# opherlieber/rltime

Measured on AMD Instinct MI355X. Metric: sampled transitions/sec (= learner steps/sec x B x T), IQN-LSTM B=512 T=80 84x84x4, higher is better.
Workload: dtype f32

## Files before the change

rltime_amd/csrc/conv_wrw.hip:

```cpp
#include "common.hpp"
#include "split3.hpp"
#include <stdlib.h>

namespace mirl {

typedef float cw_f4 __attribute__((ext_vector_type(4)));

constexpr int CW_F = 64;
constexpr int CW_MAXT = 5;

struct CwArgs {
  const float* x; const float* g; float* partial;
  int N, H, W, C, KH, KW, S, OH, OW;
  int T;
  int NT;
  int FPI;
  int KP;
  int Cp;
  int xplane;
  int gpitch;
};

template <int TPW>
__global__ void __launch_bounds__(512) __attribute__((amdgpu_waves_per_eu(2, 2)))
k_conv_wrw_b3(CwArgs a) {
  extern __shared__ __align__(16) char cw_lds[];
  uint16_t* xs = reinterpret_cast<uint16_t*>(cw_lds);
  uint16_t* gs = xs + 3 * a.xplane;
  int* tbl = reinterpret_cast<int*>(gs + 3 * CW_F * a.gpitch);
  const int tid = threadIdx.x, lane = tid & 63, wave = __builtin_amdgcn_readfirstlane(tid >> 6);
  const int j = lane & 15, kq = lane >> 4;
  const int OHW = a.OH * a.OW, fx = a.H * a.W * a.C, gplane = CW_F * a.gpitch;
  const int ksteps = a.KP >> 5;
  for (int p = tid; p < a.KP; p += 512) {
    const int f = p / OHW, r = p - f * OHW, oh = r / a.OW, ow = r - oh * a.OW;
    tbl[p] = f < a.FPI ? ((f * a.H + a.S * oh) * a.W + a.S * ow) * a.Cp : 0;
  }
  for (int o = tid; o < 3 * a.xplane / 8; o += 512) reinterpret_cast<uint4*>(xs)[o] = make_uint4(0u, 0u, 0u, 0u);
  const int nt0 = wave * TPW;
  int toff[TPW];
#pragma unroll
  for (int i = 0; i < TPW; ++i) {
    int t = (nt0 + i) * 16 + j; if (t > a.T - 1) t = a.T - 1;
    const int c = t % a.C, kk = t / a.C, kw = kk % a.KW, kh = kk / a.KW;
    toff[i] = (kh * a.W + kw) * a.Cp + c;
  }
  g3_f32x4 acc[4][TPW];
#pragma unroll
  for (int m = 0; m < 4; ++m)
#pragma unroll
    for (int i = 0; i < TPW; ++i) acc[m][i] = g3_f32x4{0.f, 0.f, 0.f, 0.f};

  const int units = (a.N + a.FPI - 1) / a.FPI;
  auto put_x = [&](const cw_f4& v, int o) {
    const float q[4] = {v.x, v.y, v.z, v.w};
    uint2 h, m, l;
    g3_split4(q, h, m, l);
    const int pix = (o * 4) / a.C, c0 = o * 4 - pix * a.C;
    uint32_t* d = reinterpret_cast<uint32_t*>(xs + pix * a.Cp + c0);
    d[0] = h.x; d[1] = h.y;
    d[a.xplane / 2] = m.x; d[a.xplane / 2 + 1] = m.y;
    d[a.xplane] = l.x; d[a.xplane + 1] = l.y;
  };
  auto load_g8 = [&](float (&q)[8], const float* gu, int item, int valid_pos) {
    const int f = item & 63, p0 = (item >> 6) * 8;
#pragma unroll
    for (int e = 0; e < 8; ++e) {
      const int p = p0 + e;
      const float t = gu[(int64_t)(p < valid_pos ? p : valid_pos - 1) * CW_F + f];
      q[e] = p < valid_pos ? t : 0.f;
    }
  };
  auto put_g8 = [&](const float (&q)[8], int item) {
    const int f = item & 63, p0 = (item >> 6) * 8;
    const float q0[4] = {q[0], q[1], q[2], q[3]}, q1[4] = {q[4], q[5], q[6], q[7]};
    uint2 h0, m0, l0, h1, m1, l1;
    g3_split4(q0, h0, m0, l0);
    g3_split4(q1, h1, m1, l1);
    uint16_t* d = gs + f * a.gpitch + p0;
    *reinterpret_cast<uint4*>(d) = make_uint4(h0.x, h0.y, h1.x, h1.y);
    *reinterpret_cast<uint4*>(d + gplane) = make_uint4(m0.x, m0.y, m1.x, m1.y);
    *reinterpret_cast<uint4*>(d + 2 * gplane) = make_uint4(l0.x, l0.y, l1.x, l1.y);
  };
  for (int u0 = blockIdx.x; u0 < units; u0 += gridDim.x) {
    const int n0 = u0 * a.FPI;
    const int frames = a.N - n0 < a.FPI ? a.N - n0 : a.FPI;
    const int xv = frames * fx / 4;
    __syncthreads();
    {
      const cw_f4* x4 = reinterpret_cast<const cw_f4*>(a.x + (int64_t)n0 * fx);
      const float* gu = a.g + (int64_t)n0 * OHW * CW_F;
      const int items = (a.KP >> 3) * CW_F, valid_pos = frames * OHW;
      constexpr int LX = 7, LG = 2;
      cw_f4 v[LX];
      float q[LG][8];
#pragma unroll
      for (int k = 0; k < LX; ++k) { const int o = tid + k * 512; v[k] = x4[o < xv ? o : xv - 1]; }
#pragma unroll
      for (int k = 0; k < LG; ++k) { const int it = tid + k * 512; load_g8(q[k], gu, it < items ? it : items - 1, valid_pos); }
#pragma unroll
      for (int k = 0; k < LX; ++k) { const int o = tid + k * 512; if (o < xv) put_x(v[k], o); }
#pragma unroll
      for (int k = 0; k < LG; ++k) { const int it = tid + k * 512; if (it < items) put_g8(q[k], it); }
      for (int o0 = tid + LX * 512; o0 < xv; o0 += 512) put_x(x4[o0], o0);
      for (int it = tid + LG * 512; it < items; it += 512) { float r[8]; load_g8(r, gu, it, valid_pos); put_g8(r, it); }
    }
    __syncthreads();
    for (int ks = 0; ks < ksteps; ++ks) {
      const int p0 = ks * 32 + kq * 8;
      int org[8];
      {
        const int4 t0 = *reinterpret_cast<const int4*>(tbl + p0), t1 = *reinterpret_cast<const int4*>(tbl + p0 + 4);
        org[0] = t0.x; org[1] = t0.y; org[2] = t0.z; org[3] = t0.w; org[4] = t1.x; org[5] = t1.y; org[6] = t1.z; org[7] = t1.w;
      }
      g3_bf16x8 af[4][3];
#pragma unroll
      for (int m = 0; m < 4; ++m)
#pragma unroll
        for (int p = 0; p < 3; ++p)
          af[m][p] = *reinterpret_cast<const g3_bf16x8*>(gs + p * gplane + (16 * m + j) * a.gpitch + p0);
      uint32_t raw[2][3][8];
      auto read_b = [&](uint32_t (&r)[3][8], int i) {
#pragma unroll
        for (int p = 0; p < 3; ++p)
#pragma unroll
          for (int e = 0; e < 8; ++e) r[p][e] = xs[p * a.xplane + org[e] + toff[i]];
      };
      read_b(raw[0], 0);
#pragma unroll
      for (int i = 0; i < TPW; ++i) {
        if (i + 1 < TPW) read_b(raw[(i + 1) & 1], i + 1);
        __builtin_amdgcn_sched_barrier(0);
        g3_bf16x8 bf[3];
#pragma unroll
        for (int p = 0; p < 3; ++p) {
          const uint32_t* r = raw[i & 1][p];
          bf[p] = __builtin_bit_cast(g3_bf16x8, make_uint4(r[0] | (r[1] << 16), r[2] | (r[3] << 16), r[4] | (r[5] << 16), r[6] | (r[7] << 16)));
        }
        constexpr int PA[6] = {2, 0, 1, 1, 0, 0};
        constexpr int PB[6] = {0, 2, 1, 0, 1, 0};
#pragma unroll
        for (int c = 0; c < 6; ++c)
#pragma unroll
          for (int m = 0; m < 4; ++m)
            acc[m][i] = __builtin_amdgcn_mfma_f32_16x16x32_bf16(af[m][PA[c]], bf[PB[c]], acc[m][i], 0, 0, 0);
        __builtin_amdgcn_sched_barrier(0);
      }
    }
  }
  float* out = a.partial + (int64_t)blockIdx.x * CW_F * a.T;
#pragma unroll
  for (int i = 0; i < TPW; ++i) {
    const int t = (nt0 + i) * 16 + j;
    if (nt0 + i < a.NT) {
#pragma unroll
      for (int m = 0; m < 4; ++m)
#pragma unroll
        for (int r = 0; r < 4; ++r) out[(int64_t)(16 * m + 4 * kq + r) * a.T + t] = acc[m][i][r];
    }
  }
}

__global__ void __launch_bounds__(256)
k_conv_wrw_reduce(const cw_f4* __restrict__ partial, int parts, int64_t n4, cw_f4* __restrict__ dw) {
  const int64_t i = (int64_t)blockIdx.x * 256 + threadIdx.x;
  if (i >= n4) return;
  cw_f4 s0 = {0.f, 0.f, 0.f, 0.f}, s1 = s0, s2 = s0, s3 = s0;
  int p = 0;
  for (; p + 4 <= parts; p += 4) {
    s0 += partial[(int64_t)p * n4 + i]; s1 += partial[(int64_t)(p + 1) * n4 + i];
    s2 += partial[(int64_t)(p + 2) * n4 + i]; s3 += partial[(int64_t)(p + 3) * n4 + i];
  }
  for (; p < parts; ++p) s0 += partial[(int64_t)p * n4 + i];
  dw[i] = (s0 + s1) + (s2 + s3);
}

static int cw_geometry(int64_t N, int H, int W, int C, int F, int KH, int KW, int S, CwArgs* a, size_t* lds, unsigned* grid) {
  if (F != CW_F || C < 4 || (C % 4) || KH < 1 || KW < 1 || S < 1 || H < KH || W < KW) return 0;
  const int T = KH * KW * C;
  if (T % 16) return 0;
  const int NT = T / 16;
  if (NT > 8 * CW_MAXT) return 0;
  const int OH = (H - KH) / S + 1, OW = (W - KW) / S + 1, OHW = OH * OW;
  if ((OHW * CW_F) % 4) return 0;
  int best = 0;
  size_t best_lds = 0;
  double best_waste = 0.0;
  for (int fpi = 1; fpi <= 4; ++fpi) {
    const int KP = (fpi * OHW + 31) / 32 * 32;
    const int xplane = (fpi * H * W * (C + 2) + 7) / 8 * 8;
    const size_t need = (size_t)3 * xplane * 2 + (size_t)3 * CW_F * (KP + 8) * 2 + (size_t)KP * 4;
    if (need > 150 * 1024) break;
    const double waste = (double)KP / (fpi * OHW);
    if (!best || waste <= best_waste + 1e-9) { best = fpi; best_lds = need; best_waste = waste; }
  }
  if (!best) return 0;
  if (a) {
    a->N = (int)N; a->H = H; a->W = W; a->C = C; a->KH = KH; a->KW = KW; a->S = S; a->OH = OH; a->OW = OW;
    a->T = T; a->NT = NT; a->FPI = best; a->KP = (best * OHW + 31) / 32 * 32;
    a->Cp = C + 2; a->xplane = (best * H * W * (C + 2) + 7) / 8 * 8; a->gpitch = a->KP + 8;
    const int64_t units = (N + best - 1) / best;
    *grid = (unsigned)(units < 256 ? units : 256);
    *lds = best_lds;
  }
  return 1;
}

}

extern "C" int mirl_conv_wrw_b3_supported(int32_t C, int32_t F, int32_t KH, int32_t KW, int32_t S, int32_t H, int32_t W) {
  return mirl::cw_geometry(1, H, W, C, F, KH, KW, S, nullptr, nullptr, nullptr);
}

extern "C" int mirl_conv_wrw_b3_scratch_bytes(int32_t C, int32_t F, int32_t KH, int32_t KW, int64_t* bytes) {
  if (!bytes || F != mirl::CW_F || C < 1 || KH < 1 || KW < 1) return mirl::fail(MIRL_ERR_ARG, "conv_wrw_b3_scratch_bytes: bad arguments");
  *bytes = (int64_t)256 * F * KH * KW * C * (int64_t)sizeof(float);
  return MIRL_OK;
}

extern "C" int mirl_conv_wrw_b3(int64_t N, int32_t H, int32_t W, int32_t C, int32_t F, int32_t KH, int32_t KW, int32_t S,
                                const float* x, const float* g, void* scratch, int64_t scratch_bytes, float* dw, void* stream) {
  using namespace mirl;
  CwArgs a;
  size_t lds = 0;
  unsigned grid = 0;
  if (N <= 0 || N >= (1LL << 30) || !x || !g || !scratch || !dw) return fail(MIRL_ERR_ARG, "bad conv_wrw_b3 arguments");
  if (!cw_geometry(N, H, W, C, F, KH, KW, S, &a, &lds, &grid)) return fail(MIRL_ERR_ARG, "conv_wrw_b3: unsupported layer shape");
  if (((uintptr_t)x % 16) || ((uintptr_t)g % 16) || ((uintptr_t)scratch % 16) || ((uintptr_t)dw % 16))
    return fail(MIRL_ERR_ARG, "conv_wrw_b3: pointers must be 16-byte aligned");
  if (scratch_bytes < (int64_t)grid * CW_F * a.T * (int64_t)sizeof(float)) return fail(MIRL_ERR_ARG, "conv_wrw_b3: scratch too small");
  a.x = x; a.g = g; a.partial = (float*)scratch;
  hipStream_t st = (hipStream_t)stream;
  const int tpw = (a.NT + 7) / 8;
  const void* fns[CW_MAXT] = {(const void*)k_conv_wrw_b3<1>, (const void*)k_conv_wrw_b3<2>, (const void*)k_conv_wrw_b3<3>,
                              (const void*)k_conv_wrw_b3<4>, (const void*)k_conv_wrw_b3<5>};
  static bool attr[CW_MAXT] = {false, false, false, false, false};
  const void* fn = fns[tpw - 1];
  if (!attr[tpw - 1]) { MIRL_HIP(hipFuncSetAttribute(fn, hipFuncAttributeMaxDynamicSharedMemorySize, 150 * 1024)); attr[tpw - 1] = true; }
  {
    ProfScope ps("k_conv_wrw_b3", 4.0 * (double)N * ((double)H * W * C + (double)a.OH * a.OW * CW_F), st,
                 2.0 * (double)N * a.OH * a.OW * CW_F * a.T);
    void* kargs[] = {(void*)&a};
    MIRL_HIP(hipLaunchKernel(fn, dim3(grid), dim3(512), kargs, lds, st));
  }
  ProfScope ps("k_conv_wrw_reduce", (double)(grid + 1) * CW_F * a.T * 4.0, st);
  const int64_t n4 = (int64_t)CW_F * a.T / 4;
  hipLaunchKernelGGL(k_conv_wrw_reduce, dim3((unsigned)((n4 + 255) / 256)), dim3(256), 0, st, reinterpret_cast<const cw_f4*>(scratch),
                     (int)grid, n4, reinterpret_cast<cw_f4*>(dw));
  MIRL_LAUNCH_CHECK();
  return MIRL_OK;
}
```

Baseline: 481,100.

## Use ds_read_tr16 transposed LDS reads and bank-conflict-aware channel padding in conv wrw

Measured after the change: 484,400 (median of 6 runs). About the same (+0.7%).

```diff
diff --git a/rltime_amd/csrc/conv_wrw.hip b/rltime_amd/csrc/conv_wrw.hip
--- a/rltime_amd/csrc/conv_wrw.hip
+++ b/rltime_amd/csrc/conv_wrw.hip
@@ -8,6 +8,7 @@
 
 constexpr int CW_F = 64;
 constexpr int CW_MAXT = 5;
+constexpr int CW_SLABS = 256;
 
 struct CwArgs {
   const float* x; const float* g; float* partial;
@@ -20,6 +21,14 @@
   int xplane;
   int gpitch;
 };
+
+typedef short cw_i16x4 __attribute__((ext_vector_type(4)));
+
+__device__ __forceinline__ uint2 cw_read_tr(const uint16_t* p) {
+  typedef __attribute__((address_space(3))) cw_i16x4 lds_i16x4;
+  const cw_i16x4 v = __builtin_amdgcn_ds_read_tr16_b64_v4i16((lds_i16x4*)(p));
+  return __builtin_bit_cast(uint2, v);
+}
 
 template <int TPW>
 __global__ void __launch_bounds__(512) __attribute__((amdgpu_waves_per_eu(2, 2)))
@@ -41,7 +50,8 @@
   int toff[TPW];
 #pragma unroll
   for (int i = 0; i < TPW; ++i) {
-    int t = (nt0 + i) * 16 + j; if (t > a.T - 1) t = a.T - 1;
+    const int nt = nt0 + i < a.NT ? nt0 + i : a.NT - 1;
+    const int t = nt * 16 + 4 * (j & 3);
     const int c = t % a.C, kk = t / a.C, kw = kk % a.KW, kh = kk / a.KW;
     toff[i] = (kh * a.W + kw) * a.Cp + c;
   }
@@ -57,10 +67,10 @@
     uint2 h, m, l;
     g3_split4(q, h, m, l);
     const int pix = (o * 4) / a.C, c0 = o * 4 - pix * a.C;
-    uint32_t* d = reinterpret_cast<uint32_t*>(xs + pix * a.Cp + c0);
-    d[0] = h.x; d[1] = h.y;
-    d[a.xplane / 2] = m.x; d[a.xplane / 2 + 1] = m.y;
-    d[a.xplane] = l.x; d[a.xplane + 1] = l.y;
+    uint2* d = reinterpret_cast<uint2*>(xs + pix * a.Cp + c0);
+    d[0] = h;
+    d[a.xplane / 4] = m;
+    d[a.xplane / 2] = l;
   };
   auto load_g8 = [&](float (&q)[8], const float* gu, int item, int valid_pos) {
     const int f = item & 63, p0 = (item >> 6) * 8;
@@ -108,35 +118,27 @@
     __syncthreads();
     for (int ks = 0; ks < ksteps; ++ks) {
       const int p0 = ks * 32 + kq * 8;
-      int org[8];
-      {
-        const int4 t0 = *reinterpret_cast<const int4*>(tbl + p0), t1 = *reinterpret_cast<const int4*>(tbl + p0 + 4);
-        org[0] = t0.x; org[1] = t0.y; org[2] = t0.z; org[3] = t0.w; org[4] = t1.x; org[5] = t1.y; org[6] = t1.z; org[7] = t1.w;
-      }
+      const int o0 = tbl[p0 + (j >> 2)], o1 = tbl[p0 + 4 + (j >> 2)];
       g3_bf16x8 af[4][3];
 #pragma unroll
       for (int m = 0; m < 4; ++m)
 #pragma unroll
         for (int p = 0; p < 3; ++p)
           af[m][p] = *reinterpret_cast<const g3_bf16x8*>(gs + p * gplane + (16 * m + j) * a.gpitch + p0);
-      uint32_t raw[2][3][8];
-      auto read_b = [&](uint32_t (&r)[3][8], int i) {
-#pragma unroll
-        for (int p = 0; p < 3; ++p)
-#pragma unroll
-          for (int e = 0; e < 8; ++e) r[p][e] = xs[p * a.xplane + org[e] + toff[i]];
+      g3_bf16x8 bb[2][3];
+      auto read_b = [&](g3_bf16x8 (&b)[3], int i) {
+#pragma unroll
+        for (int p = 0; p < 3; ++p) {
+          const uint2 lo = cw_read_tr(xs + p * a.xplane + o0 + toff[i]), hi = cw_read_tr(xs + p * a.xplane + o1 + toff[i]);
+          b[p] = __builtin_bit_cast(g3_bf16x8, make_uint4(lo.x, lo.y, hi.x, hi.y));
+        }
       };
-      read_b(raw[0], 0);
+      read_b(bb[0], 0);
 #pragma unroll
       for (int i = 0; i < TPW; ++i) {
-        if (i + 1 < TPW) read_b(raw[(i + 1) & 1], i + 1);
+        if (i + 1 < TPW) read_b(bb[(i + 1) & 1], i + 1);
         __builtin_amdgcn_sched_barrier(0);
-        g3_bf16x8 bf[3];
-#pragma unroll
-        for (int p = 0; p < 3; ++p) {
-          const uint32_t* r = raw[i & 1][p];
-          bf[p] = __builtin_bit_cast(g3_bf16x8, make_uint4(r[0] | (r[1] << 16), r[2] | (r[3] << 16), r[4] | (r[5] << 16), r[6] | (r[7] << 16)));
-        }
+        const g3_bf16x8 (&bf)[3] = bb[i & 1];
         constexpr int PA[6] = {2, 0, 1, 1, 0, 0};
         constexpr int PB[6] = {0, 2, 1, 0, 1, 0};
 #pragma unroll
@@ -175,6 +177,22 @@
   dw[i] = (s0 + s1) + (s2 + s3);
 }
 
+static int cw_read_cycles(int fpi, int H, int W, int S, int OW, int OHW, int KP, int Cp) {
+  int total = 0;
+  for (int p0 = 0; p0 < KP; p0 += 16)
+    for (int sub = 0; sub < 2; ++sub) {
+      int cnt[64] = {0}, worst = 0;
+      for (int k = 0; k < 2; ++k)
+        for (int q = 0; q < 4; ++q) {
+          const int p = p0 + 8 * k + 4 * sub + q, f = p / OHW, r = p - f * OHW, oh = r / OW, ow = r - oh * OW;
+          const int org = f < fpi ? ((f * H + S * oh) * W + S * ow) * Cp : 0;
+          for (int b = 0; b < 8; ++b) { const int bank = (org / 2 + b) & 63; if (++cnt[bank] > worst) worst = cnt[bank]; }
+        }
+      total += worst;
+    }
+  return total;
+}
+
 static int cw_geometry(int64_t N, int H, int W, int C, int F, int KH, int KW, int S, CwArgs* a, size_t* lds, unsigned* grid) {
   if (F != CW_F || C < 4 || (C % 4) || KH < 1 || KW < 1 || S < 1 || H < KH || W < KW) return 0;
   const int T = KH * KW * C;
@@ -183,24 +201,35 @@
   if (NT > 8 * CW_MAXT) return 0;
   const int OH = (H - KH) / S + 1, OW = (W - KW) / S + 1, OHW = OH * OW;
   if ((OHW * CW_F) % 4) return 0;
-  int best = 0;
+  auto need = [&](int fpi, int Cp) {
+    const int KP = (fpi * OHW + 31) / 32 * 32;
+    const int xplane = (fpi * H * W * Cp + 7) / 8 * 8;
+    return (size_t)3 * xplane * 2 + (size_t)3 * CW_F * (KP + 8) * 2 + (size_t)KP * 4;
+  };
+  int best = 0, best_cp = 0;
   size_t best_lds = 0;
   double best_waste = 0.0;
   for (int fpi = 1; fpi <= 4; ++fpi) {
+    if (need(fpi, C) > 150 * 1024) break;
     const int KP = (fpi * OHW + 31) / 32 * 32;
-    const int xplane = (fpi * H * W * (C + 2) + 7) / 8 * 8;
-    const size_t need = (size_t)3 * xplane * 2 + (size_t)3 * CW_F * (KP + 8) * 2 + (size_t)KP * 4;
-    if (need > 150 * 1024) break;
     const double waste = (double)KP / (fpi * OHW);
-    if (!best || waste <= best_waste + 1e-9) { best = fpi; best_lds = need; best_waste = waste; }
+    if (best && waste > best_waste + 1e-9) continue;
+    int cp = C, cyc = -1;
+    for (int k = 0; k < 8; ++k) {
+      const int Cp = C + 4 * k;
+      if (need(fpi, Cp) > 150 * 1024) break;
+      const int c = cw_read_cycles(fpi, H, W, S, OW, OHW, KP, Cp);
+      if (cyc < 0 || c < cyc) { cyc = c; cp = Cp; }
+    }
+    best = fpi; best_cp = cp; best_lds = need(fpi, cp); best_waste = waste;
   }
   if (!best) return 0;
   if (a) {
     a->N = (int)N; a->H = H; a->W = W; a->C = C; a->KH = KH; a->KW = KW; a->S = S; a->OH = OH; a->OW = OW;
     a->T = T; a->NT = NT; a->FPI = best; a->KP = (best * OHW + 31) / 32 * 32;
-    a->Cp = C + 2; a->xplane = (best * H * W * (C + 2) + 7) / 8 * 8; a->gpitch = a->KP + 8;
+    a->Cp = best_cp; a->xplane = (best * H * W * best_cp + 7) / 8 * 8; a->gpitch = a->KP + 8;
     const int64_t units = (N + best - 1) / best;
-    *grid = (unsigned)(units < 256 ? units : 256);
+    *grid = (unsigned)(units < CW_SLABS ? units : CW_SLABS);
     *lds = best_lds;
   }
   return 1;
@@ -214,7 +243,7 @@
 
 extern "C" int mirl_conv_wrw_b3_scratch_bytes(int32_t C, int32_t F, int32_t KH, int32_t KW, int64_t* bytes) {
   if (!bytes || F != mirl::CW_F || C < 1 || KH < 1 || KW < 1) return mirl::fail(MIRL_ERR_ARG, "conv_wrw_b3_scratch_bytes: bad arguments");
-  *bytes = (int64_t)256 * F * KH * KW * C * (int64_t)sizeof(float);
+  *bytes = (int64_t)mirl::CW_SLABS * F * KH * KW * C * (int64_t)sizeof(float);
   return MIRL_OK;
 }
 
```
